# frgfm/Holocron

Hardware: NVIDIA H100
Metric: images/sec RepVGG-A0 224^2 bf16 train (higher is better)
Workload: dtype bf16

## Files before the change

### holocron_b200/csrc/conv_rows.cu

```cuda
#include "conv_common.cuh"

namespace {

using namespace tc;
using namespace conv;

struct RowsParams {
  int N, H, W, Cin, Cout;
  int Wp;
  int SR;
  int NSUB;
  int TRO;
  int CB;
  int ksteps_last;
  int tiles_per_img, num_tiles;
  int nstages;
  int stage_bytes;
  int cb_bytes;
  int ecb_bytes;
  int w_tap_bytes;
  int out_pitch;
  int act;
  int nextra;
  __nv_bfloat16* y;
  const float* bias;
  const __nv_bfloat16* residual;
  float* stats;
};

template <int BN>
__global__ void __launch_bounds__(kThreads, 1)
conv_rows_kernel(const __grid_constant__ CUtensorMap tmX, const __grid_constant__ CUtensorMap tmW,
                 const __grid_constant__ CUtensorMap tmXe0, const __grid_constant__ CUtensorMap tmWe0,
                 const __grid_constant__ CUtensorMap tmXe1, const __grid_constant__ CUtensorMap tmWe1, const RowsParams p) {
  extern __shared__ __align__(1024) uint8_t smem_raw[];
  uint8_t* smem = reinterpret_cast<uint8_t*>((reinterpret_cast<uintptr_t>(smem_raw) + 1023) & ~uintptr_t(1023));
  uint8_t* wsm = smem;
  uint8_t* stage0 = wsm + (size_t)(9 + p.nextra) * p.CB * p.w_tap_bytes;
  uint8_t* sout = stage0 + (size_t)p.nstages * p.stage_bytes;
  const size_t sout_bytes = ((size_t)128 * p.out_pitch + 15) & ~size_t(15);
  uint64_t* bars = reinterpret_cast<uint64_t*>(sout + sout_bytes);
  uint64_t* full_bar = bars;
  uint64_t* empty_bar = bars + 2;
  uint64_t* w_bar = bars + 4;

  const int warp = threadIdx.x >> 5, lane = threadIdx.x & 31;
  if (warp == 0 && lane == 0) {
    prefetch_tmap(&tmX);
    prefetch_tmap(&tmW);
    for (int i = 0; i < 2; ++i) { mbar_init(&full_bar[i], 1); mbar_init(&empty_bar[i], kConsumers / 32); }
    mbar_init(w_bar, 1);
    fence_barrier_init();
  }
  __syncthreads();

  if (warp < 4) {
    if (warp == 0 && lane == 0) {
      prefetch_tmap(&tmXe0); prefetch_tmap(&tmWe0); prefetch_tmap(&tmXe1); prefetch_tmap(&tmWe1);
      mbar_arrive_expect_tx(w_bar, (uint32_t)((9 + p.nextra) * p.CB * BN * 128));
      for (int tap = 0; tap < 9; ++tap)
        for (int cb = 0; cb < p.CB; ++cb)
          tma_load_3d(&tmW, w_bar, wsm + (size_t)(tap * p.CB + cb) * p.w_tap_bytes, cb * 64, tap, 0);
      for (int e = 0; e < p.nextra; ++e)
        for (int cb = 0; cb < p.CB; ++cb)
          tma_load_3d(e == 0 ? &tmWe0 : &tmWe1, w_bar, wsm + (size_t)((9 + e) * p.CB + cb) * p.w_tap_bytes, cb * 64, 0, 0);
      const uint32_t tx = (uint32_t)(p.CB * ((p.TRO + 2) + p.nextra * p.TRO) * p.Wp * 128);
      int it = 0;
      for (int tile = blockIdx.x; tile < p.num_tiles; tile += gridDim.x, ++it) {
        const int n = tile / p.tiles_per_img, p0 = (tile % p.tiles_per_img) * p.TRO;
        const Ring ring = Ring::at(it, p.nstages);
        mbar_wait(&empty_bar[ring.stage], ring.phase ^ 1);
        mbar_arrive_expect_tx(&full_bar[ring.stage], tx);
        for (int b = 0; b <= p.nextra; ++b) {
          const CUtensorMap* tm = b == 0 ? &tmX : (b == 1 ? &tmXe0 : &tmXe1);
          const int h0 = b == 0 ? p0 - 1 : p0;
          for (int cb = 0; cb < p.CB; ++cb) {
            tma_load_4d(tm, &full_bar[ring.stage],
                        stage0 + (size_t)ring.stage * p.stage_bytes +
                            (size_t)p.CB * (b ? p.cb_bytes + (b - 1) * p.ecb_bytes : 0) +
                            (size_t)cb * (b ? p.ecb_bytes : p.cb_bytes),
                        cb * 64, -1, h0, n);
          }
        }
      }
    }
    return;
  }

  const int et = threadIdx.x - 128;
  const int wg = et >> 7;
  const int frow = 64 * wg + frag_row(et & 127);
  const int fcol = frag_col(et & 127);
  const uint32_t dhi = desc_hi(1024);
  const uint32_t w_lo0 = desc_lo(smem_u32(wsm), 16);
  const uint32_t w_tap_lo = (uint32_t)p.w_tap_bytes >> 4;
  const uint32_t cb_lo = (uint32_t)p.cb_bytes >> 4;
  const uint32_t ecb_lo = (uint32_t)p.ecb_bytes >> 4;
  const int chunks_per_row = BN / 8;
  const int npairs = BN >> 1, rgs = kConsumers / npairs;
  const int st_rg = et / npairs, st_pr = et - st_rg * npairs;
  const bool st_on = p.stats != nullptr && st_rg < rgs;
  float4 stat = make_float4(0.f, 0.f, 0.f, 0.f);
  float acc[64];
  mbar_wait(w_bar, 0);
  int it = 0;
  for (int tile = blockIdx.x; tile < p.num_tiles; tile += gridDim.x, ++it) {
    const int n = tile / p.tiles_per_img, p0 = (tile % p.tiles_per_img) * p.TRO;
    const Ring ring = Ring::at(it, p.nstages);
    mbar_wait(&full_bar[ring.stage], ring.phase);
    const uint32_t s_lo =
        desc_lo(smem_u32(stage0 + (size_t)ring.stage * p.stage_bytes), 16) + (uint32_t)wg * ((64 * 128) >> 4);
    for (int sub = 0; sub < p.NSUB; ++sub) {
#pragma unroll 1
      for (int tap = 0; tap < 9; ++tap) {
        const int r = tap / 3, s = tap % 3;
        uint32_t a_lo = s_lo + (uint32_t)(((sub * p.SR + r) * p.Wp + s) * 8);
        uint32_t b_lo = w_lo0 + (uint32_t)(tap * p.CB) * w_tap_lo;
        for (int cb = 0; cb < p.CB; ++cb) {
          const int ks = (cb == p.CB - 1) ? p.ksteps_last : 4;
          wgmma_group_ks<BN, 0, 0>(ks, acc, a_lo, b_lo, 2, dhi, (tap | cb) ? 1u : 0u);
          a_lo += cb_lo;
          b_lo += w_tap_lo;
        }
      }
      for (int e = 0; e < p.nextra; ++e) {
        uint32_t a_lo = s_lo + (uint32_t)p.CB * (cb_lo + e * ecb_lo) + (uint32_t)((sub * p.SR * p.Wp + 1) * 8);
        uint32_t b_lo = w_lo0 + (uint32_t)((9 + e) * p.CB) * w_tap_lo;
        for (int cb = 0; cb < p.CB; ++cb) {
          const int ks = (cb == p.CB - 1) ? p.ksteps_last : 4;
          wgmma_group_ks<BN, 0, 0>(ks, acc, a_lo, b_lo, 2, dhi, 1u);
          a_lo += ecb_lo;
          b_lo += w_tap_lo;
        }
      }
      wgmma_wait<0>();
      fence_regs(acc);
      if (sub == p.NSUB - 1 && lane == 0) mbar_arrive(&empty_bar[ring.stage]);

      consumer_sync();
#pragma unroll
      for (int j = 0; j < 16; ++j) {
        const int col = 8 * j + fcol;
        if (col < BN) {
#pragma unroll
          for (int h = 0; h < 2; ++h) {
            float f0 = acc[4 * j + 2 * h], f1 = acc[4 * j + 2 * h + 1];
            if (p.bias) { f0 += __ldg(p.bias + col); f1 += __ldg(p.bias + col + 1); }
            if (p.act == 1 && !p.residual) { f0 = hb::relu_nan(f0); f1 = hb::relu_nan(f1); }
            *reinterpret_cast<__nv_bfloat162*>(sout + (size_t)(frow + 8 * h) * p.out_pitch + col * 2) =
                __floats2bfloat162_rn(f0, f1);
          }
        }
      }
      consumer_sync();
      const int row0 = p0 + sub * p.SR;
      const int rows_valid = max(0, min(p.SR, min(p.H, p0 + p.TRO) - row0));
      const int total = rows_valid * p.W * chunks_per_row;
      int pix0 = et / chunks_per_row;
      int c8 = et - pix0 * chunks_per_row;
      int i = pix0 / p.W, q = pix0 - i * p.W;
      const int dpix = kConsumers / chunks_per_row, dc = kConsumers - dpix * chunks_per_row;
      const int di = dpix / p.W, dq = dpix - di * p.W;
      for (int ch = et; ch < total; ch += kConsumers) {
        uint4 val = *reinterpret_cast<const uint4*>(sout + (size_t)(i * p.Wp + q) * p.out_pitch + c8 * 16);
        const size_t off = ((size_t)(n * p.H + row0 + i) * p.W + q) * p.Cout + c8 * 8;
        if (p.residual) {
          const uint4 rv = *reinterpret_cast<const uint4*>(p.residual + off);
          add_residual16(val, rv, p.act == 1);
        }
        *reinterpret_cast<uint4*>(p.y + off) = val;
        c8 += dc; q += dq; i += di;
        if (c8 >= chunks_per_row) { c8 -= chunks_per_row; ++q; }
        if (q >= p.W) { q -= p.W; ++i; }
      }
      if (st_on && !p.residual) {
        const int npix = rows_valid * p.W;
        int si = st_rg / p.W, sq = st_rg - si * p.W;
        const int sdi = rgs / p.W, sdq = rgs - sdi * p.W;
        const uint8_t* sp = sout + st_pr * 4;
        for (int v = st_rg; v < npix; v += rgs) {
          accum_pair(stat, sp + (size_t)(si * p.Wp + sq) * p.out_pitch);
          sq += sdq; si += sdi;
          if (sq >= p.W) { sq -= p.W; ++si; }
        }
      }
    }
  }
  if (p.stats) {
    consumer_sync();
    float4* scratch = reinterpret_cast<float4*>(sout);
    scratch[et] = stat;
    consumer_sync();
    if (et < 2 * BN) {
      const int c = et % BN, half = et / BN;
      store_stats(p.stats, blockIdx.x * 2 + half, p.Cout, c,
                  half == 0 ? fold_stats(scratch, rgs, npairs, c) : make_float2(0.f, 0.f));
    }
  }
}

}

int hb_conv_rows_try(const void* x, const void* w, void* y, const float* bias, const void* residual, int N, int H, int W,
                     int Cin, int Cout, int act, int num_ctas, cudaStream_t stream, int nextra, const void* const* xe,
                     const void* const* we, float* stats, int* stat_slots) {
  constexpr int kNo = (int)cudaErrorNotSupported;
  if (stats && (residual || !stat_slots)) return kNo;
  if (Cout % 16 != 0 || Cout > 128 || Cin % 8 != 0 || Cin > 128) return kNo;
  const int Wp = W + 2;
  if (Wp > 128 || W < 8 || nextra < 0 || nextra > 2) return kNo;
  RowsParams p{};
  p.N = N; p.H = H; p.W = W; p.Cin = Cin; p.Cout = Cout; p.Wp = Wp; p.nextra = nextra;
  p.SR = 128 / Wp;
  p.CB = (Cin + 63) / 64;
  const int last = Cin - (p.CB - 1) * 64;
  p.ksteps_last = (last + 15) / 16;
  p.w_tap_bytes = ((Cout * 128) + 1023) & ~1023;
  p.out_pitch = Cout * 2 + 16;
  const int w_bytes = (9 + nextra) * p.CB * p.w_tap_bytes;
  const int out_bytes = (((128 * p.out_pitch + 15) & ~15) + 1023) & ~1023;
  const int budget = 222 * 1024 - w_bytes - out_bytes - 256;
  const int max_rows_needed = (H + p.SR - 1) / p.SR;
  int nsub = 0;
  for (int nst = 2; nst >= 1 && nsub < 1; --nst) {
    for (nsub = max_rows_needed < 8 ? max_rows_needed : 8; nsub >= 1; --nsub) {
      const int tro = nsub * p.SR;
      const int reach = (((nsub - 1) * p.SR + 2) * Wp + 2 + 128) * 128;
      const int rows = (tro + 2) * Wp * 128;
      const int need = ((rows > reach ? rows : reach) + 1023) & ~1023;
      const int ereach = ((nsub - 1) * p.SR * Wp + 1 + 128) * 128, erows = tro * Wp * 128;
      const int eneed = ((erows > ereach ? erows : ereach) + 1023) & ~1023;
      if (nst * p.CB * (need + nextra * eneed) <= budget) {
        p.nstages = nst; p.cb_bytes = need; p.ecb_bytes = eneed;
        break;
      }
    }
  }
  if (nsub < 1) return kNo;
  p.NSUB = nsub;
  p.TRO = nsub * p.SR;
  p.stage_bytes = p.CB * (p.cb_bytes + nextra * p.ecb_bytes);
  p.tiles_per_img = (H + p.TRO - 1) / p.TRO;
  p.num_tiles = N * p.tiles_per_img;
  p.act = act;
  p.y = (__nv_bfloat16*)y; p.bias = bias; p.residual = (const __nv_bfloat16*)residual;
  p.stats = stats;

  CUtensorMap tmX, tmW, tmXe[2], tmWe[2];
  if (tmap::encode_nhwc_box(&tmX, x, N, H, W, Cin, Wp, p.TRO + 2)) return kNo;
  if (tmap::encode_krsc_slab(&tmW, w, Cout, 9, Cin, Cout)) return kNo;
  for (int e = 0; e < 2; ++e) {
    const void* xs = e < nextra ? xe[e] : x;
    const void* ws = e < nextra ? we[e] : w;
    if (!hb::aligned16(xs) || !hb::aligned16(ws)) return kNo;
    if (tmap::encode_nhwc_box(&tmXe[e], xs, N, H, W, Cin, Wp, p.TRO)) return kNo;
    if (tmap::encode_krsc_slab(&tmWe[e], ws, Cout, 1, Cin, Cout)) return kNo;
  }
  const size_t smem_bytes = (size_t)w_bytes + (size_t)p.nstages * p.stage_bytes + out_bytes + 64 + 1024;
  if (smem_bytes > 227 * 1024) return kNo;
  int grid = num_ctas > 0 ? num_ctas : HB_NUM_SMS;
  if (grid > p.num_tiles) grid = p.num_tiles;
  if (stat_slots) *stat_slots = 2 * grid;
  return (int)dispatch_width<16, 128>(Cout, [&](auto bn) {
    return launch<conv_rows_kernel<decltype(bn)::value>>(grid, smem_bytes, stream, tmX, tmW, tmXe[0], tmWe[0], tmXe[1],
                                                          tmWe[1], p);
  });
}

extern "C" {

int hb_conv3x3_accum_bf16(const void* x, const void* w, const void* xe0, const void* we0, const void* xe1, const void* we1,
                          int nextra, void* y, int N, int H, int W, int Cin, int Cout, int num_ctas, void* stream) {
  const void* xe[2] = {xe0, xe1};
  const void* we[2] = {we0, we1};
  if (!hb::aligned16(x) || !hb::aligned16(w) || !hb::aligned16(y)) return (int)cudaErrorMisalignedAddress;
  return hb_conv_rows_try(x, w, y, nullptr, nullptr, N, H, W, Cin, Cout, 0, num_ctas, (cudaStream_t)stream, nextra, xe, we,
                          nullptr, nullptr);
}

}
```

Before: 9332.

## Warp-specialize conv epilogue with double-buffered output staging and paired wgmma chains

The previously idle producer warps 1-3 become a dedicated store group that drains a double-buffered shared-memory output tile to global memory, adds the residual and accumulates batch-norm stats. Handoff to the consumer warpgroups uses mbarriers, so the consumers can start the next sub-tile's MMAs while the previous one is being written out. For BN<=64, two sub-tiles are issued together as interleaved wgmma chains that share the B descriptor, to increase MMA issue density. The extra output buffer uses more shared memory, which can shrink the input stage budget. Cout is now capped at 112, so 128-channel layers fall back to another path.

```diff
diff --git a/holocron_b200/csrc/conv_rows.cu b/holocron_b200/csrc/conv_rows.cu
--- a/holocron_b200/csrc/conv_rows.cu
+++ b/holocron_b200/csrc/conv_rows.cu
@@ -4,6 +4,32 @@
 
 using namespace tc;
 using namespace conv;
+
+constexpr int kStoreThreads = 96;
+__device__ __forceinline__ void store_sync() { asm volatile("bar.sync 2, 96;" ::: "memory"); }
+
+template <int N, int KS>
+__device__ __forceinline__ void wgmma_group2(float* d0, float* d1, uint32_t a0, uint32_t a1, uint32_t b_lo, uint32_t dhi,
+                                             uint32_t scale_first) {
+  wgmma_fence();
+#pragma unroll
+  for (int k = 0; k < KS; ++k) {
+    const uint64_t b = make_desc(b_lo + 2 * k, dhi);
+    wgmma<N, 0, 0>(d0, make_desc(a0 + 2 * k, dhi), b, k ? 1u : scale_first);
+    wgmma<N, 0, 0>(d1, make_desc(a1 + 2 * k, dhi), b, k ? 1u : scale_first);
+  }
+  wgmma_commit();
+}
+template <int N>
+__device__ __forceinline__ void wgmma_group2_ks(int ks, float* d0, float* d1, uint32_t a0, uint32_t a1, uint32_t b_lo,
+                                                uint32_t dhi, uint32_t scale_first) {
+  switch (ks) {
+    case 1: wgmma_group2<N, 1>(d0, d1, a0, a1, b_lo, dhi, scale_first); break;
+    case 2: wgmma_group2<N, 2>(d0, d1, a0, a1, b_lo, dhi, scale_first); break;
+    case 3: wgmma_group2<N, 3>(d0, d1, a0, a1, b_lo, dhi, scale_first); break;
+    default: wgmma_group2<N, 4>(d0, d1, a0, a1, b_lo, dhi, scale_first); break;
+  }
+}
 
 struct RowsParams {
   int N, H, W, Cin, Cout;
@@ -37,25 +63,32 @@
   uint8_t* smem = reinterpret_cast<uint8_t*>((reinterpret_cast<uintptr_t>(smem_raw) + 1023) & ~uintptr_t(1023));
   uint8_t* wsm = smem;
   uint8_t* stage0 = wsm + (size_t)(9 + p.nextra) * p.CB * p.w_tap_bytes;
-  uint8_t* sout = stage0 + (size_t)p.nstages * p.stage_bytes;
-  const size_t sout_bytes = ((size_t)128 * p.out_pitch + 15) & ~size_t(15);
-  uint64_t* bars = reinterpret_cast<uint64_t*>(sout + sout_bytes);
+  uint8_t* sout0 = stage0 + (size_t)p.nstages * p.stage_bytes;
+  const size_t sout_bytes = ((size_t)128 * p.out_pitch + 1023) & ~size_t(1023);
+  uint64_t* bars = reinterpret_cast<uint64_t*>(sout0 + 2 * sout_bytes);
   uint64_t* full_bar = bars;
   uint64_t* empty_bar = bars + 2;
   uint64_t* w_bar = bars + 4;
+  uint64_t* out_full = bars + 5;
+  uint64_t* out_empty = bars + 7;
 
   const int warp = threadIdx.x >> 5, lane = threadIdx.x & 31;
   if (warp == 0 && lane == 0) {
     prefetch_tmap(&tmX);
     prefetch_tmap(&tmW);
-    for (int i = 0; i < 2; ++i) { mbar_init(&full_bar[i], 1); mbar_init(&empty_bar[i], kConsumers / 32); }
+    for (int i = 0; i < 2; ++i) {
+      mbar_init(&full_bar[i], 1);
+      mbar_init(&empty_bar[i], kConsumers / 32);
+      mbar_init(&out_full[i], kConsumers / 32);
+      mbar_init(&out_empty[i], kStoreThreads / 32);
+    }
     mbar_init(w_bar, 1);
     fence_barrier_init();
   }
   __syncthreads();
 
-  if (warp < 4) {
-    if (warp == 0 && lane == 0) {
+  if (warp == 0) {
+    if (lane == 0) {
       prefetch_tmap(&tmXe0); prefetch_tmap(&tmWe0); prefetch_tmap(&tmXe1); prefetch_tmap(&tmWe1);
       mbar_arrive_expect_tx(w_bar, (uint32_t)((9 + p.nextra) * p.CB * BN * 128));
       for (int tap = 0; tap < 9; ++tap)
@@ -87,6 +120,68 @@
     return;
   }
 
+  if (warp < 4) {
+    const int st = threadIdx.x - 32;
+    const int chunks_per_row = BN / 8;
+    const int npairs = BN >> 1, rgs = kStoreThreads / npairs;
+    const int st_rg = st / npairs, st_pr = st - st_rg * npairs;
+    const bool st_on = p.stats != nullptr && st_rg < rgs;
+    float4 stat = make_float4(0.f, 0.f, 0.f, 0.f);
+    const int dpix = kStoreThreads / chunks_per_row, dc = kStoreThreads - dpix * chunks_per_row;
+    const int di = dpix / p.W, dq = dpix - di * p.W;
+    const int sdi = rgs / p.W, sdq = rgs - sdi * p.W;
+    int k = 0;
+    for (int tile = blockIdx.x; tile < p.num_tiles; tile += gridDim.x) {
+      const int n = tile / p.tiles_per_img, p0 = (tile % p.tiles_per_img) * p.TRO;
+      for (int sub = 0; sub < p.NSUB; ++sub, ++k) {
+        const uint8_t* sout = sout0 + (size_t)(k & 1) * sout_bytes;
+        mbar_wait(&out_full[k & 1], (uint32_t)(k >> 1) & 1);
+        const int row0 = p0 + sub * p.SR;
+        const int rows_valid = max(0, min(p.SR, min(p.H, p0 + p.TRO) - row0));
+        const int total = rows_valid * p.W * chunks_per_row;
+        int pix0 = st / chunks_per_row;
+        int c8 = st - pix0 * chunks_per_row;
+        int i = pix0 / p.W, q = pix0 - i * p.W;
+        for (int ch = st; ch < total; ch += kStoreThreads) {
+          uint4 val = *reinterpret_cast<const uint4*>(sout + (size_t)(i * p.Wp + q) * p.out_pitch + c8 * 16);
+          const size_t off = ((size_t)(n * p.H + row0 + i) * p.W + q) * p.Cout + c8 * 8;
+          if (p.residual) {
+            const uint4 rv = *reinterpret_cast<const uint4*>(p.residual + off);
+            add_residual16(val, rv, p.act == 1);
+          }
+          *reinterpret_cast<uint4*>(p.y + off) = val;
+          c8 += dc; q += dq; i += di;
+          if (c8 >= chunks_per_row) { c8 -= chunks_per_row; ++q; }
+          if (q >= p.W) { q -= p.W; ++i; }
+        }
+        if (st_on && !p.residual) {
+          const int npix = rows_valid * p.W;
+          int si = st_rg / p.W, sq = st_rg - si * p.W;
+          const uint8_t* sp = sout + st_pr * 4;
+          for (int v = st_rg; v < npix; v += rgs) {
+            accum_pair(stat, sp + (size_t)(si * p.Wp + sq) * p.out_pitch);
+            sq += sdq; si += sdi;
+            if (sq >= p.W) { sq -= p.W; ++si; }
+          }
+        }
+        __syncwarp();
+        if (lane == 0) mbar_arrive(&out_empty[k & 1]);
+      }
+    }
+    if (p.stats) {
+      store_sync();
+      float4* scratch = reinterpret_cast<float4*>(sout0);
+      scratch[st] = stat;
+      store_sync();
+      for (int e = st; e < 2 * BN; e += kStoreThreads) {
+        const int c = e % BN, half = e / BN;
+        store_stats(p.stats, blockIdx.x * 2 + half, p.Cout, c,
+                    half == 0 ? fold_stats(scratch, rgs, npairs, c) : make_float2(0.f, 0.f));
+      }
+    }
+    return;
+  }
+
   const int et = threadIdx.x - 128;
   const int wg = et >> 7;
   const int frow = 64 * wg + frag_row(et & 127);
@@ -96,29 +191,34 @@
   const uint32_t w_tap_lo = (uint32_t)p.w_tap_bytes >> 4;
   const uint32_t cb_lo = (uint32_t)p.cb_bytes >> 4;
   const uint32_t ecb_lo = (uint32_t)p.ecb_bytes >> 4;
-  const int chunks_per_row = BN / 8;
-  const int npairs = BN >> 1, rgs = kConsumers / npairs;
-  const int st_rg = et / npairs, st_pr = et - st_rg * npairs;
-  const bool st_on = p.stats != nullptr && st_rg < rgs;
-  float4 stat = make_float4(0.f, 0.f, 0.f, 0.f);
-  float acc[64];
+  constexpr int kChains = BN <= 64 ? 2 : 1;
+  float acc[kChains][BN / 2];
+  const uint32_t sub_lo = (uint32_t)(p.SR * p.Wp * 8);
   mbar_wait(w_bar, 0);
-  int it = 0;
+  int it = 0, k = 0;
   for (int tile = blockIdx.x; tile < p.num_tiles; tile += gridDim.x, ++it) {
-    const int n = tile / p.tiles_per_img, p0 = (tile % p.tiles_per_img) * p.TRO;
     const Ring ring = Ring::at(it, p.nstages);
     mbar_wait(&full_bar[ring.stage], ring.phase);
     const uint32_t s_lo =
         desc_lo(smem_u32(stage0 + (size_t)ring.stage * p.stage_bytes), 16) + (uint32_t)wg * ((64 * 128) >> 4);
-    for (int sub = 0; sub < p.NSUB; ++sub) {
+    for (int sub = 0; sub < p.NSUB; sub += kChains) {
+      const bool pair = kChains == 2 && sub + 1 < p.NSUB;
+      auto issue = [&](int ks, uint32_t a_lo, uint32_t b_lo, uint32_t scale_first) {
+        if constexpr (kChains == 2) {
+          if (pair) {
+            wgmma_group2_ks<BN>(ks, acc[0], acc[kChains - 1], a_lo, a_lo + sub_lo, b_lo, dhi, scale_first);
+            return;
+          }
+        }
+        wgmma_group_ks<BN, 0, 0>(ks, acc[0], a_lo, b_lo, 2, dhi, scale_first);
+      };
 #pragma unroll 1
       for (int tap = 0; tap < 9; ++tap) {
         const int r = tap / 3, s = tap % 3;
         uint32_t a_lo = s_lo + (uint32_t)(((sub * p.SR + r) * p.Wp + s) * 8);
         uint32_t b_lo = w_lo0 + (uint32_t)(tap * p.CB) * w_tap_lo;
         for (int cb = 0; cb < p.CB; ++cb) {
-          const int ks = (cb == p.CB - 1) ? p.ksteps_last : 4;
-          wgmma_group_ks<BN, 0, 0>(ks, acc, a_lo, b_lo, 2, dhi, (tap | cb) ? 1u : 0u);
+          issue((cb == p.CB - 1) ? p.ksteps_last : 4, a_lo, b_lo, (tap | cb) ? 1u : 0u);
           a_lo += cb_lo;
           b_lo += w_tap_lo;
         }
@@ -127,74 +227,39 @@
         uint32_t a_lo = s_lo + (uint32_t)p.CB * (cb_lo + e * ecb_lo) + (uint32_t)((sub * p.SR * p.Wp + 1) * 8);
         uint32_t b_lo = w_lo0 + (uint32_t)((9 + e) * p.CB) * w_tap_lo;
         for (int cb = 0; cb < p.CB; ++cb) {
-          const int ks = (cb == p.CB - 1) ? p.ksteps_last : 4;
-          wgmma_group_ks<BN, 0, 0>(ks, acc, a_lo, b_lo, 2, dhi, 1u);
+          issue((cb == p.CB - 1) ? p.ksteps_last : 4, a_lo, b_lo, 1u);
           a_lo += ecb_lo;
           b_lo += w_tap_lo;
         }
       }
       wgmma_wait<0>();
-      fence_regs(acc);
-      if (sub == p.NSUB - 1 && lane == 0) mbar_arrive(&empty_bar[ring.stage]);
-
-      consumer_sync();
-#pragma unroll
-      for (int j = 0; j < 16; ++j) {
-        const int col = 8 * j + fcol;
-        if (col < BN) {
-#pragma unroll
-          for (int h = 0; h < 2; ++h) {
-            float f0 = acc[4 * j + 2 * h], f1 = acc[4 * j + 2 * h + 1];
-            if (p.bias) { f0 += __ldg(p.bias + col); f1 += __ldg(p.bias + col + 1); }
-            if (p.act == 1 && !p.residual) { f0 = hb::relu_nan(f0); f1 = hb::relu_nan(f1); }
-            *reinterpret_cast<__nv_bfloat162*>(sout + (size_t)(frow + 8 * h) * p.out_pitch + col * 2) =
-                __floats2bfloat162_rn(f0, f1);
-          }
-        }
-      }
-      consumer_sync();
-      const int row0 = p0 + sub * p.SR;
-      const int rows_valid = max(0, min(p.SR, min(p.H, p0 + p.TRO) - row0));
-      const int total = rows_valid * p.W * chunks_per_row;
-      int pix0 = et / chunks_per_row;
-      int c8 = et - pix0 * chunks_per_row;
-      int i = pix0 / p.W, q = pix0 - i * p.W;
-      const int dpix = kConsumers / chunks_per_row, dc = kConsumers - dpix * chunks_per_row;
-      const int di = dpix / p.W, dq = dpix - di * p.W;
-      for (int ch = et; ch < total; ch += kConsumers) {
-        uint4 val = *reinterpret_cast<const uint4*>(sout + (size_t)(i * p.Wp + q) * p.out_pitch + c8 * 16);
-        const size_t off = ((size_t)(n * p.H + row0 + i) * p.W + q) * p.Cout + c8 * 8;
-        if (p.residual) {
-          const uint4 rv = *reinterpret_cast<const uint4*>(p.residual + off);
-          add_residual16(val, rv, p.act == 1);
-        }
-        *reinterpret_cast<uint4*>(p.y + off) = val;
-        c8 += dc; q += dq; i += di;
-        if (c8 >= chunks_per_row) { c8 -= chunks_per_row; ++q; }
-        if (q >= p.W) { q -= p.W; ++i; }
-      }
-      if (st_on && !p.residual) {
-        const int npix = rows_valid * p.W;
-        int si = st_rg / p.W, sq = st_rg - si * p.W;
-        const int sdi = rgs / p.W, sdq = rgs - sdi * p.W;
-        const uint8_t* sp = sout + st_pr * 4;
-        for (int v = st_rg; v < npix; v += rgs) {
-          accum_pair(stat, sp + (size_t)(si * p.Wp + sq) * p.out_pitch);
-          sq += sdq; si += sdi;
-          if (sq >= p.W) { sq -= p.W; ++si; }
-        }
-      }
-    }
-  }
-  if (p.stats) {
-    consumer_sync();
-    float4* scratch = reinterpret_cast<float4*>(sout);
-    scratch[et] = stat;
-    consumer_sync();
-    if (et < 2 * BN) {
-      const int c = et % BN, half = et / BN;
-      store_stats(p.stats, blockIdx.x * 2 + half, p.Cout, c,
-                  half == 0 ? fold_stats(scratch, rgs, npairs, c) : make_float2(0.f, 0.f));
+#pragma unroll
+      for (int c = 0; c < kChains; ++c) fence_regs(acc[c]);
+      if (sub + kChains >= p.NSUB && lane == 0) mbar_arrive(&empty_bar[ring.stage]);
+
+#pragma unroll
+      for (int c = 0; c < kChains; ++c) {
+        if (c == 1 && !pair) break;
+        uint8_t* sout = sout0 + (size_t)(k & 1) * sout_bytes;
+        mbar_wait(&out_empty[k & 1], ((uint32_t)(k >> 1) & 1) ^ 1);
+#pragma unroll
+        for (int j = 0; j < 16; ++j) {
+          const int col = 8 * j + fcol;
+          if (col < BN) {
+#pragma unroll
+            for (int h = 0; h < 2; ++h) {
+              float f0 = acc[c][4 * j + 2 * h], f1 = acc[c][4 * j + 2 * h + 1];
+              if (p.bias) { f0 += __ldg(p.bias + col); f1 += __ldg(p.bias + col + 1); }
+              if (p.act == 1 && !p.residual) { f0 = hb::relu_nan(f0); f1 = hb::relu_nan(f1); }
+              *reinterpret_cast<__nv_bfloat162*>(sout + (size_t)(frow + 8 * h) * p.out_pitch + col * 2) =
+                  __floats2bfloat162_rn(f0, f1);
+            }
+          }
+        }
+        __syncwarp();
+        if (lane == 0) mbar_arrive(&out_full[k & 1]);
+        ++k;
+      }
     }
   }
 }
@@ -206,7 +271,7 @@
                      const void* const* we, float* stats, int* stat_slots) {
   constexpr int kNo = (int)cudaErrorNotSupported;
   if (stats && (residual || !stat_slots)) return kNo;
-  if (Cout % 16 != 0 || Cout > 128 || Cin % 8 != 0 || Cin > 128) return kNo;
+  if (Cout % 16 != 0 || Cout > 112 || Cin % 8 != 0 || Cin > 128) return kNo;
   const int Wp = W + 2;
   if (Wp > 128 || W < 8 || nextra < 0 || nextra > 2) return kNo;
   RowsParams p{};
@@ -219,7 +284,8 @@
   p.out_pitch = Cout * 2 + 16;
   const int w_bytes = (9 + nextra) * p.CB * p.w_tap_bytes;
   const int out_bytes = (((128 * p.out_pitch + 15) & ~15) + 1023) & ~1023;
-  const int budget = 222 * 1024 - w_bytes - out_bytes - 256;
+  constexpr int kBarBytes = 128, kAlignBytes = 1024;
+  const int budget = 227 * 1024 - w_bytes - 2 * out_bytes - kBarBytes - kAlignBytes;
   const int max_rows_needed = (H + p.SR - 1) / p.SR;
   int nsub = 0;
   for (int nst = 2; nst >= 1 && nsub < 1; --nst) {
@@ -256,12 +322,12 @@
     if (tmap::encode_nhwc_box(&tmXe[e], xs, N, H, W, Cin, Wp, p.TRO)) return kNo;
     if (tmap::encode_krsc_slab(&tmWe[e], ws, Cout, 1, Cin, Cout)) return kNo;
   }
-  const size_t smem_bytes = (size_t)w_bytes + (size_t)p.nstages * p.stage_bytes + out_bytes + 64 + 1024;
+  const size_t smem_bytes = (size_t)w_bytes + (size_t)p.nstages * p.stage_bytes + 2 * out_bytes + kBarBytes + kAlignBytes;
   if (smem_bytes > 227 * 1024) return kNo;
   int grid = num_ctas > 0 ? num_ctas : HB_NUM_SMS;
   if (grid > p.num_tiles) grid = p.num_tiles;
   if (stat_slots) *stat_slots = 2 * grid;
-  return (int)dispatch_width<16, 128>(Cout, [&](auto bn) {
+  return (int)dispatch_width<16, 112>(Cout, [&](auto bn) {
     return launch<conv_rows_kernel<decltype(bn)::value>>(grid, smem_bytes, stream, tmX, tmW, tmXe[0], tmWe[0], tmXe[1],
                                                           tmWe[1], p);
   });
```

New measurement: 9572 (median of 6 runs). +2.6%, better.
